# stripe/rainier

Hardware: NVIDIA H100
Metric: leapfrog_steps_x_chains_per_sec (higher is better)
Workload: dtype f64

## Files before the change

rainier_b200/csrc/rn_sampler.cuh:

```cuda
#ifndef RN_SAMPLER_CUH
#define RN_SAMPLER_CUH


#if RN_MASS_MAX >= 1
#define RN_TS_NMASS RN_N
#else
#define RN_TS_NMASS 0
#endif
#if RN_ENABLE_EHMC
#define RN_TS_NSNAP RN_N
#else
#define RN_TS_NSNAP 0
#endif
#ifndef RN_TS_RESTORE
#define RN_TS_RESTORE 0
#endif
#if RN_TS_RESTORE
#define RN_TS_NREST (2 * RN_N + 1)
#else
#define RN_TS_NREST 0
#endif
#define RN_TS_P 0
#define RN_TS_MASS (RN_N + 1)
#define RN_TS_SNAP (RN_TS_MASS + RN_TS_NMASS)
#define RN_TS_STAT (RN_TS_SNAP + RN_TS_NSNAP)
#define RN_TS_HOT (RN_TS_STAT + 5)
#define RN_TS_REST (RN_TS_HOT + 4)
#define RN_TS_DOUBLES (RN_TS_REST + RN_TS_NREST)
#define RN_TS_INTS 10
struct RnTs {
  double* d;
  int* i;
  unsigned bs;
};
#ifdef RN_HOST_EMULATION
static thread_local double rn_ts_mem_d[RN_TS_DOUBLES];
static thread_local int rn_ts_mem_i[RN_TS_INTS];
RN_DEVICE RnTs rn_ts_get() { return RnTs{rn_ts_mem_d, rn_ts_mem_i, 1u}; }
#define RN_STCS(ptr, v) (*(ptr) = (v))
#else
extern __shared__ double rn_ts_mem[];
RN_DEVICE RnTs rn_ts_get() {
  RnTs T;
#ifdef RN_BLOCK_DIM
  T.bs = RN_BLOCK_DIM;
#else
  T.bs = blockDim.x;
#endif
  T.d = rn_ts_mem + threadIdx.x;
  T.i = (int*)(rn_ts_mem + (size_t)RN_TS_DOUBLES * blockDim.x) + threadIdx.x;
  return T;
}
#define RN_STCS(ptr, v) __stcs((ptr), (v))
#endif
#define RN_TSD(slot) T.d[(unsigned)(slot) * T.bs]
#define RN_TSI(slot) T.i[(unsigned)(slot) * T.bs]
#ifndef RN_X_P_REGS
#define RN_X_P_REGS 1
#endif
#ifndef RN_X_NORMALS
#define RN_X_NORMALS 3
#endif
#define RN_Z(i) RN_TSD(RN_TS_P + (i))
#if RN_X_P_REGS
#define RN_P(i) s.p[i]
#else
#define RN_P(i) RN_TSD(RN_TS_P + (i))
#endif
#define RN_MASSD(i) RN_TSD(RN_TS_MASS + (i))
#define RN_SNAP_P(i) RN_TSD(RN_TS_SNAP + (i))
#define RN_ST_E_MEAN RN_TSD(RN_TS_STAT + 0)
#define RN_ST_E_RAW RN_TSD(RN_TS_STAT + 1)
#define RN_ST_TRANS2 RN_TSD(RN_TS_STAT + 2)
#define RN_ST_GRADS RN_TSD(RN_TS_STAT + 3)
#define RN_ST_STEPS RN_TSD(RN_TS_STAT + 4)
#define RN_ST_ITERS RN_TSI(0)
#define RN_ST_ACCEPTED RN_TSI(1)
#define RN_ST_E_N RN_TSI(2)
#define RN_ST_RING_I(r) RN_TSI(3 + (r))
#define RN_ST_RING_FULL(r) RN_TSI(6 + (r))
#define RN_TS_PREV_H RN_TSD(RN_TS_HOT + 2)
#define RN_TS_START_H RN_TSD(RN_TS_HOT + 3)
#define RN_REST_Q(i) RN_TSD(RN_TS_REST + (i))
#define RN_REST_G(i) RN_TSD(RN_TS_REST + RN_N + (i))
#define RN_REST_U RN_TSD(RN_TS_REST + 2 * RN_N)

struct RnIt {
  int grads, steps, err;
};

RN_DEVICE RnRng rn_rng_unpark(const RnTs& T) {
  RnRng r;
  r.seed = rn_d2ll(RN_TSD(RN_TS_HOT + 0));
  r.nng = RN_TSD(RN_TS_HOT + 1);
  r.have = RN_TSI(9);
  return r;
}
RN_DEVICE void rn_rng_park(const RnTs& T, const RnRng& r) {
  RN_TSD(RN_TS_HOT + 0) = rn_ll2d(r.seed);
  RN_TSD(RN_TS_HOT + 1) = r.nng;
  RN_TSI(9) = r.have;
}

RN_DEVICE void rn_ring_add(const RnArgs& A, int c, const RnTs& T, int which, double value) {
  int i = RN_ST_RING_I(which) + 1;
  if (i == A.stats_window) {
    RN_ST_RING_FULL(which) = 1;
    i = 0;
  }
  RN_ST_RING_I(which) = i;
  RN_STCS(&RN_AT(A.st_rings, which * A.stats_window + i, c), value);
}

struct RnPQ {
  double q[RN_N], g[RN_N];
  double U;
#if RN_X_P_REGS
  double p[RN_N];
#endif
};

RN_DEVICE double rn_velocity_i(const RnArgs& A, int c, const RnTs& T, const RnPQ& s, int kind, int i) {
  (void)s;
  (void)T;
  (void)A;
  (void)c;
#if RN_MASS_MAX >= 2
  if (kind == 2) {
    double y = 0.0;
    for (int j = 0; j < RN_N; j++) y += RN_P(j) * RN_AT(A.mass, i * RN_N + j, c);
    return y;
  }
#endif
#if RN_MASS_MAX >= 1
  if (kind == 1) return RN_P(i) * RN_MASSD(i);
#endif
  (void)kind;
  return RN_P(i);
}

RN_DEVICE double rn_energy(const RnArgs& A, int c, const RnTs& T, const RnPQ& s, int kind, double U) {
  double k = 0.0;
#if RN_MASS_MAX >= 2
  if (kind == 2) {
    for (int i = 0; i < RN_N; i++) k += (rn_velocity_i(A, c, T, s, 2, i) * RN_P(i));
    return U + k / 2.0;
  }
#endif
  RN_UNROLL
  for (int i = 0; i < RN_N; i++) k += (rn_velocity_i(A, c, T, s, kind, i) * RN_P(i));
  return U + k / 2.0;
}

RN_DEVICE double rn_log_accept(double deltaH) {
  if (deltaH != deltaH) return -RN_INF;
  return rn_jmin0(-deltaH);
}


RN_DEVICE void rn_update(const RnArgs& A, RnPQ& s, RnIt& S) {
  double dens;
  rn_density(s.q, dens, s.g, A.data, S.err);
  s.U = dens * -1;
  S.grads += 1;
}
RN_DEVICE void rn_full_ps(const RnTs& T, RnPQ& s, double stepSize, RnIt& S) {
  (void)T;
  S.grads += 1;
  RN_UNROLL
  for (int i = 0; i < RN_N; i++) RN_P(i) += stepSize * s.g[i];
}
RN_DEVICE void rn_new_qs(const RnArgs& A, int c, const RnTs& T, int kind, RnPQ& s, double stepSize) {
#if RN_MASS_MAX >= 2
  if (kind == 2) {
    for (int i = 0; i < RN_N; i++) s.q[i] += (stepSize * rn_velocity_i(A, c, T, s, 2, i));
    return;
  }
#endif
  RN_UNROLL
  for (int i = 0; i < RN_N; i++) s.q[i] += (stepSize * rn_velocity_i(A, c, T, s, kind, i));
}
RN_DEVICE void rn_leapfrog(const RnArgs& A, int c, const RnTs& T, int kind, RnPQ& s, int l, double stepSize, RnIt& S) {
  rn_full_ps(T, s, stepSize / 2.0, S);
  for (int i = 0;;) {
    rn_new_qs(A, c, T, kind, s, stepSize);
    rn_update(A, s, S);
    if (++i >= l) break;
    rn_full_ps(T, s, stepSize, S);
  }
  rn_full_ps(T, s, stepSize / 2.0, S);
}
RN_DEVICE void rn_take_steps(const RnArgs& A, int c, const RnTs& T, int kind, RnPQ& s, int l, double stepSize, RnIt& S) {
  rn_ring_add(A, c, T, 0, stepSize);
  rn_leapfrog(A, c, T, kind, s, l, stepSize, S);
  S.steps += l;
}

RN_DEVICE void rn_draw_normals(const RnTs& T, RnRng& rng) {
#if RN_X_NORMALS == 2
  for (int i = 0; i < RN_N; i++) RN_Z(i) = rn_normal(rng);
  return;
#endif
  int i0 = 0;
  if (rng.have) {
    rng.have = 0;
    RN_Z(0) = rng.nng;
    i0 = 1;
  }
  const int npairs = (RN_N - i0 + 1) / 2;
#ifndef RN_X_POLAR2
#define RN_X_POLAR2 1
#endif
#if RN_X_POLAR2
  for (int k = 0; k < npairs;) {
    double a1, a2, b1, b2;
    rn_i64 seed4, seed8;
    rn_polar_attempt2(rng, a1, a2, b1, b2, seed4, seed8);
    const double sa = a1 * a1 + a2 * a2, sb = b1 * b1 + b2 * b2;
    const bool oka = !(sa >= 1 || sa == 0);
    const int kb = k + (oka ? 1 : 0);
    const bool needb = kb < npairs;
    const bool okb = needb && !(sb >= 1 || sb == 0);
    if (oka) {
      RN_Z(i0 + 2 * k) = a1;
      RN_Z(i0 + 2 * k + 1) = a2;
    }
    if (okb) {
      RN_Z(i0 + 2 * kb) = b1;
      RN_Z(i0 + 2 * kb + 1) = b2;
    }
    rng.seed = needb ? seed8 : seed4;
    k = kb + (okb ? 1 : 0);
  }
#else
  for (int k = 0; k < npairs;) {
    double v1, v2;
    rn_polar_attempt(rng, v1, v2);
    const double s = v1 * v1 + v2 * v2;
    if (!(s >= 1 || s == 0)) {
      RN_Z(i0 + 2 * k) = v1;
      RN_Z(i0 + 2 * k + 1) = v2;
      k += 1;
    }
  }
#endif
#if RN_X_NORMALS == 4 && RN_X_SPEC && !defined(RN_FAST_MATH) && !(defined(RN_X_LIBM_PLAIN) && RN_X_LIBM_PLAIN)
#pragma unroll 1
  for (int k = 0; k < npairs; k += 2) {
    const int ia = i0 + 2 * k, ib = i0 + 2 * (k + 1 < npairs ? k + 1 : k);
    const double a1 = RN_Z(ia), a2 = RN_Z(ia + 1), b1 = RN_Z(ib), b2 = RN_Z(ib + 1);
    const double sa = a1 * a1 + a2 * a2, sb = b1 * b1 + b2 * b2;
    bool oka, okb;
    double la = rn_strict_log_try(sa, oka), lb = rn_strict_log_try(sb, okb);
    if (!(oka && okb)) {
      la = rn_strict_log_full(sa);
      lb = rn_strict_log_full(sb);
    }
    const double ma = rn_sqrt_nc(rn_div_nc(-2 * la, sa)), mb = rn_sqrt_nc(rn_div_nc(-2 * lb, sb));
    RN_Z(ia) = a1 * ma;
    if (ia + 1 < RN_N) {
      RN_Z(ia + 1) = a2 * ma;
    } else {
      rng.nng = a2 * ma;
      rng.have = 1;
    }
    RN_Z(ib) = b1 * mb;
    if (ib + 1 < RN_N) {
      RN_Z(ib + 1) = b2 * mb;
    } else {
      rng.nng = b2 * mb;
      rng.have = 1;
    }
  }
  return;
#endif
#if RN_X_NORMALS == 1
#pragma unroll 1
#elif RN_X_NORMALS == 3
#pragma unroll 2
#endif
  for (int k = 0; k < npairs; k++) {
    const int i = i0 + 2 * k;
    const double v1 = RN_Z(i), v2 = RN_Z(i + 1);
    const double s = v1 * v1 + v2 * v2;
    const double multiplier = rn_polar_multiplier(s);
    RN_Z(i) = v1 * multiplier;
    if (i + 1 < RN_N) {
      RN_Z(i + 1) = v2 * multiplier;
    } else {
      rng.nng = v2 * multiplier;
      rng.have = 1;
    }
  }
}

RN_DEVICE void rn_initialize_ps(const RnArgs& A, int c, const RnTs& T, RnPQ& s, int kind, RnRng& rng) {
  (void)A;
  (void)c;
  (void)kind;
  (void)s;
  rn_draw_normals(T, rng);
#if RN_X_P_REGS
  RN_UNROLL
  for (int i = 0; i < RN_N; i++) s.p[i] = RN_Z(i);
#endif
#if RN_MASS_MAX >= 2
  if (kind == 2) {
    int i = RN_N - 1;
    int m = ((i + 1) * (i + 2)) / 2 - 1;
    while (i >= 0) {
      int j = RN_N - 1;
      double dot = 0.0;
      while (j > i) {
        dot += RN_Z(j) * RN_AT(A.chol, m, c);
        j -= 1;
        m -= 1;
      }
      RN_Z(i) = (RN_Z(i) - dot) / RN_AT(A.chol, m, c);
      i -= 1;
      m -= 1;
    }
#if RN_X_P_REGS
    for (int k = 0; k < RN_N; k++) s.p[k] = RN_Z(k);
#endif
    return;
  }
#endif
#if RN_MASS_MAX >= 1
  if (kind == 1) {
    RN_UNROLL
    for (int i = 0; i < RN_N; i++) RN_P(i) = RN_P(i) / sqrt(RN_MASSD(i));
    return;
  }
#endif
}

RN_DEVICE void rn_load_mass(const RnArgs& A, int c, const RnTs& T, int kind) {
  (void)A;
  (void)c;
  (void)T;
  (void)kind;
#if RN_MASS_MAX >= 1
  if (kind == 1) {
    RN_UNROLL
    for (int i = 0; i < RN_N; i++) RN_MASSD(i) = RN_AT(A.mass, i, c);
  }
#endif
}

RN_DEVICE void rn_load_stats(const RnArgs& A, int c, const RnTs& T) {
  RN_ST_GRADS = rn_ll2d(A.st_grads[c]);
  RN_ST_STEPS = rn_ll2d(A.st_steps[c]);
  RN_ST_ITERS = A.st_iters[c];
  RN_ST_ACCEPTED = A.st_accepted[c];
  RN_ST_E_MEAN = RN_AT(A.st_energy, 0, c);
  RN_ST_E_RAW = RN_AT(A.st_energy, 1, c);
  RN_ST_TRANS2 = RN_AT(A.st_energy, 2, c);
  RN_ST_E_N = A.st_energy_n[c];
  for (int r = 0; r < 3; r++) {
    RN_ST_RING_I(r) = RN_AT(A.st_ring_i, r, c);
    RN_ST_RING_FULL(r) = RN_AT(A.st_ring_full, r, c);
  }
}
RN_DEVICE void rn_store_stats(const RnArgs& A, int c, const RnTs& T, int err) {
  A.st_grads[c] = rn_d2ll(RN_ST_GRADS);
  A.st_steps[c] = rn_d2ll(RN_ST_STEPS);
  A.st_iters[c] = RN_ST_ITERS;
  A.st_accepted[c] = RN_ST_ACCEPTED;
  if (err) A.st_err[c] |= err;
  RN_AT(A.st_energy, 0, c) = RN_ST_E_MEAN;
  RN_AT(A.st_energy, 1, c) = RN_ST_E_RAW;
  RN_AT(A.st_energy, 2, c) = RN_ST_TRANS2;
  A.st_energy_n[c] = RN_ST_E_N;
  for (int r = 0; r < 3; r++) {
    RN_AT(A.st_ring_i, r, c) = RN_ST_RING_I(r);
    RN_AT(A.st_ring_full, r, c) = RN_ST_RING_FULL(r);
  }
}
RN_DEVICE void rn_fold(const RnTs& T, RnIt& S) {
  RN_ST_GRADS = rn_ll2d(rn_d2ll(RN_ST_GRADS) + (rn_i64)S.grads);
  RN_ST_STEPS = rn_ll2d(rn_d2ll(RN_ST_STEPS) + (rn_i64)S.steps);
  S.grads = 0;
  S.steps = 0;
}

RN_GLOBAL void rn_k_init(const RnArgs A) {
  const int c = (int)(blockIdx.x * blockDim.x + threadIdx.x);
  if (c >= A.chains) return;
  const RnTs T = rn_ts_get();
  RnRng rng;
  rng.seed = A.rng_seed[c];
  rng.nng = A.rng_nng[c];
  rng.have = A.rng_have[c];
  rn_load_stats(A, c, T);
  RnIt S;
  S.grads = 0;
  S.steps = 0;
  S.err = 0;

  RnPQ s;
  rn_draw_normals(T, rng);
  RN_UNROLL
  for (int i = 0; i < RN_N; i++) s.q[i] = RN_Z(i);
  rn_update(A, s, S);
  double cq[RN_N], cg[RN_N];
  const double cU = s.U;
  RN_UNROLL
  for (int i = 0; i < RN_N; i++) {
    cq[i] = s.q[i];
    cg[i] = s.g[i];
  }
  rn_initialize_ps(A, c, T, s, 0, rng);
  RN_UNROLL
  for (int i = 0; i < RN_N; i++) RN_AT(A.params, i, c) = RN_P(i);

  double stepSize;
  if (A.step_tuner == 0) {
    const double H0 = rn_energy(A, c, T, s, 0, cU);
    stepSize = 1.0;
    double lap;
    rn_leapfrog(A, c, T, 0, s, 1, stepSize, S);
    lap = rn_log_accept(rn_energy(A, c, T, s, 0, s.U) - H0);
    const double exponent = (lap > -RN_LN2) ? 1.0 : -1.0;
    const double doubleOrHalf = (exponent > 0) ? 2.0 : 0.5;
#if RN_STEP_POOL
    int log2Step = 0;
#endif
    while (stepSize != 0.0 && (exponent * lap > -exponent * RN_LN2)) {
      stepSize *= doubleOrHalf;
#if RN_STEP_POOL
      log2Step += (exponent > 0) ? 1 : -1;
#endif
      RN_UNROLL
      for (int i = 0; i < RN_N; i++) {
        RN_P(i) = RN_AT(A.params, i, c);
        s.q[i] = cq[i];
        s.g[i] = cg[i];
      }
      s.U = cU;
      rn_leapfrog(A, c, T, 0, s, 1, stepSize, S);
      lap = rn_log_accept(rn_energy(A, c, T, s, 0, s.U) - H0);
    }
    rn_da_apply(stepSize, RN_AT(A.da, 1, c), RN_AT(A.da, 2, c), RN_AT(A.da, 3, c), RN_AT(A.da, 4, c), A.da_iter[c]);
#if RN_STEP_POOL
    rn_pool_add_initial_step(A.step_acc, log2Step);
#endif
  } else {
    stepSize = A.static_step;
  }
  RN_AT(A.da, 0, c) = stepSize;

  RN_UNROLL
  for (int i = 0; i < RN_N; i++) {
    RN_AT(A.params, RN_N + i, c) = cq[i];
    RN_AT(A.grad, i, c) = cg[i];
  }
  RN_AT(A.params, 2 * RN_N, c) = cU;
  A.rng_seed[c] = rng.seed;
  A.rng_nng[c] = rng.nng;
  A.rng_have[c] = rng.have;
  rn_fold(T, S);
  rn_store_stats(A, c, T, S.err);
}

enum { RN_P_IN_PARAMS = 0, RN_P_IN_REGS = 1, RN_P_IN_Z = 2 };
RN_DEVICE void rn_store_momentum(const RnArgs& A, int c, const RnTs& T, const RnPQ& s, int where) {
  (void)s;
  if (where == RN_P_IN_PARAMS) return;
  RN_UNROLL
  for (int i = 0; i < RN_N; i++) RN_AT(A.params, i, c) = where == RN_P_IN_REGS ? RN_P(i) : RN_Z(i);
}

template <int PHASE>
RN_DEVICE void rn_iterate(const RnArgs& A) {
  const int c = A.chain_begin + (int)(blockIdx.x * blockDim.x + threadIdx.x);
  if (c >= A.chain_end) return;
  const RnTs T = rn_ts_get();
  {
    RnRng rng;
    rng.seed = A.rng_seed[c];
    rng.nng = A.rng_nng[c];
    rng.have = A.rng_have[c];
    rn_rng_park(T, rng);
  }
  rn_load_stats(A, c, T);
  RnIt S;
  S.grads = 0;
  S.steps = 0;
  S.err = 0;
#if RN_MASS_MAX >= 1
  int kind = A.mass_kind;
#else
  constexpr int kind = 0;
#endif
  rn_load_mass(A, c, T, kind);

  double stepSize = RN_AT(A.da, 0, c);
  if (PHASE == 1 && A.step_tuner == 0) stepSize = rn_exp(RN_AT(A.da, 2, c));
  int win_size = A.win_size, win_i = A.win_i, win_j = A.win_j, est_samples = A.est_samples;
#if RN_ENABLE_EHMC
  int ring_i = 0, ring_full = 0;
  if (A.sampler == 1) {
    ring_i = A.ring_i[c];
    ring_full = A.ring_full[c];
  }
#endif
  bool havePrevH = false;

#ifndef RN_X_KEEP_STATE
#define RN_X_KEEP_STATE 1
#endif
#define RN_KEEP_P_LATE (RN_X_KEEP_STATE && RN_X_P_REGS)
#define RN_REST_ON_CHIP (RN_X_KEEP_STATE && RN_TS_RESTORE)
#if RN_REST_ON_CHIP
#define RN_X0(i) RN_REST_Q(i)
  int p_at = RN_P_IN_PARAMS;
#else
#define RN_X0(i) RN_AT(A.params, RN_N + (i), c)
#endif
  RnPQ s;
#if RN_X_KEEP_STATE
  RN_UNROLL
  for (int i = 0; i < RN_N; i++) {
    s.q[i] = RN_AT(A.params, RN_N + i, c);
    s.g[i] = RN_AT(A.grad, i, c);
  }
  s.U = RN_AT(A.params, 2 * RN_N, c);
#endif

  for (int it = 0; it < A.n_iter; it++) {
#if RN_X_KEEP_STATE
    const double cU = s.U;
#else
    const double cU = RN_AT(A.params, 2 * RN_N, c);
#endif
    if (!havePrevH) {
      RN_UNROLL
      for (int i = 0; i < RN_N; i++) RN_P(i) = RN_AT(A.params, i, c);
      RN_TS_PREV_H = rn_energy(A, c, T, s, kind, cU);
    }
    {
      RnRng rng = rn_rng_unpark(T);
      rn_initialize_ps(A, c, T, s, kind, rng);
      rn_rng_park(T, rng);
    }
#if RN_X_KEEP_STATE
    if (!(RN_KEEP_P_LATE && kind == 0)) {
      RN_UNROLL
      for (int i = 0; i < RN_N; i++) RN_AT(A.params, i, c) = RN_P(i);
    }
#else
    RN_UNROLL
    for (int i = 0; i < RN_N; i++) {
      RN_AT(A.params, i, c) = RN_P(i);
      s.q[i] = RN_AT(A.params, RN_N + i, c);
      s.g[i] = RN_AT(A.grad, i, c);
    }
#endif
    s.U = cU;
    RN_TS_START_H = rn_energy(A, c, T, s, kind, cU);
#if RN_REST_ON_CHIP
    RN_UNROLL
    for (int i = 0; i < RN_N; i++) {
      RN_REST_Q(i) = s.q[i];
      RN_REST_G(i) = s.g[i];
    }
    RN_REST_U = cU;
#endif
    const double usedStep = stepSize;

    if (A.sampler == 0) {
      rn_take_steps(A, c, T, kind, s, A.n_steps, stepSize, S);
    }
#if RN_ENABLE_EHMC
    else {
      bool count = false;
      if (PHASE == 0 && !ring_full) count = true;
      else if (PHASE == 0) {
        RnRng rng = rn_rng_unpark(T);
        count = rn_uniform(rng) < A.p_count;
        rn_rng_park(T, rng);
      }
      if (count) {
        RnPQ snap;
        int l = 0;
        for (;;) {
          double out = 0.0;
          RN_UNROLL
          for (int i = 0; i < RN_N; i++) out += (s.q[i] - RN_X0(i)) * RN_P(i);
          const bool uturn = (out != out) ? true : (out < 0);
          if (uturn || !(l < A.max_steps)) break;
          l += 1;
          rn_take_steps(A, c, T, kind, s, 1, stepSize, S);
          if (l == A.min_steps) {
            snap = s;
#if !(RN_X_P_REGS)
            RN_UNROLL
            for (int i = 0; i < RN_N; i++) RN_SNAP_P(i) = RN_P(i);
#endif
          }
        }
        if (l < A.min_steps) {
          rn_take_steps(A, c, T, kind, s, A.min_steps - l, stepSize, S);
        } else {
          s = snap;
#if !(RN_X_P_REGS)
          RN_UNROLL
          for (int i = 0; i < RN_N; i++) RN_P(i) = RN_SNAP_P(i);
#endif
        }
        ring_i += 1;
        if (ring_i == A.buf_size) ring_full = 1;
        ring_i = ring_i % A.buf_size;
        RN_AT(A.ring, ring_i, c) = (double)l;
      } else {
        RnRng rng = rn_rng_unpark(T);
        const int idx = ring_full ? rn_rng_int(rng, A.buf_size) : rn_rng_int(rng, ring_i + 1);
        rn_rng_park(T, rng);
        const int nsteps = rn_d2i(RN_AT(A.ring, idx, c));
        rn_take_steps(A, c, T, kind, s, nsteps, stepSize, S);
      }
    }
#endif

    const double endH = rn_energy(A, c, T, s, kind, s.U);
    const double startH = RN_TS_START_H;
    const double deltaH = endH - startH;
    const double a = rn_log_accept(deltaH);
    bool accept;
    {
      RnRng rng = rn_rng_unpark(T);
      accept = a > rn_log(rn_uniform(rng));
      rn_rng_park(T, rng);
    }
    double eH;
    if (accept) {
#if RN_REST_ON_CHIP
      p_at = RN_P_IN_REGS;
#else
      RN_UNROLL
      for (int i = 0; i < RN_N; i++) {
        RN_AT(A.params, i, c) = RN_P(i);
        RN_AT(A.params, RN_N + i, c) = s.q[i];
        RN_AT(A.grad, i, c) = s.g[i];
      }
      RN_AT(A.params, 2 * RN_N, c) = s.U;
#endif
      eH = endH;
      RN_ST_ACCEPTED += 1;
    } else {
#if RN_REST_ON_CHIP
      RN_UNROLL
      for (int i = 0; i < RN_N; i++) {
        s.q[i] = RN_REST_Q(i);
        s.g[i] = RN_REST_G(i);
      }
      s.U = RN_REST_U;
      p_at = (RN_KEEP_P_LATE && kind == 0) ? RN_P_IN_Z : RN_P_IN_PARAMS;
#else
      RN_UNROLL
      for (int i = 0; i < RN_N; i++) s.q[i] = RN_AT(A.params, RN_N + i, c);
#if RN_X_KEEP_STATE
      RN_UNROLL
      for (int i = 0; i < RN_N; i++) s.g[i] = RN_AT(A.grad, i, c);
      s.U = RN_AT(A.params, 2 * RN_N, c);
      if (RN_KEEP_P_LATE && kind == 0) {
        RN_UNROLL
        for (int i = 0; i < RN_N; i++) RN_AT(A.params, i, c) = RN_Z(i);
      }
#endif
#endif
      eH = startH;
    }
    {
      const int e_n = RN_ST_E_N + 1;
      RN_ST_E_N = e_n;
      double e_mean = RN_ST_E_MEAN;
      const double oldDiff = eH - e_mean;
      e_mean += (oldDiff / (double)e_n);
      RN_ST_E_MEAN = e_mean;
      const double newDiff = eH - e_mean;
      RN_ST_E_RAW += oldDiff * newDiff;
      const double d = eH - RN_TS_PREV_H;
      RN_ST_TRANS2 += d * d;
    }
    RN_TS_PREV_H = eH;
    havePrevH = true;
    RN_ST_ITERS += 1;
    rn_ring_add(A, c, T, 1, rn_exp(a));
    rn_ring_add(A, c, T, 2, (double)S.grads);

    if (A.trace) {
      double* tr = A.trace + (size_t)it * 4 * (size_t)A.chains;
      tr[0 * (size_t)A.chains + c] = a;
      tr[1 * (size_t)A.chains + c] = accept ? 1.0 : 0.0;
      tr[2 * (size_t)A.chains + c] = usedStep;
      tr[3 * (size_t)A.chains + c] = (double)S.steps;
    }
    rn_fold(T, S);

    if (PHASE == 0) {
#if RN_STEP_POOL
      if (A.step_tuner == 0) rn_pool_add(A.step_acc + it, rn_pool_quantise(rn_exp(a)));
#else
      if (A.step_tuner == 0) {
        const double newAcceptanceProb = rn_exp(a);
        const int daIter = A.da_iter[c] + 1;
        A.da_iter[c] = daIter;
        const double avgErrorMultiplier = 1.0 / ((double)daIter + 10);
        const double stepSizeMultiplier = rn_pow((double)daIter, -0.75);
        const double avgError = ((1.0 - avgErrorMultiplier) * RN_AT(A.da, 3, c) + (avgErrorMultiplier * (A.delta - newAcceptanceProb)));
        RN_AT(A.da, 3, c) = avgError;
        const double logStepSize = (RN_AT(A.da, 4, c) - (avgError * sqrt((double)daIter) / 0.05));
        RN_AT(A.da, 1, c) = logStepSize;
        RN_AT(A.da, 2, c) = (stepSizeMultiplier * logStepSize + (1.0 - stepSizeMultiplier) * RN_AT(A.da, 2, c));
        stepSize = rn_exp(logStepSize);
      }
#endif
#if RN_MASS_MAX >= 1
      if (A.mass_tuner == 1 || A.mass_tuner == 2) {
        win_j += 1;
        if (A.adaptation == 1) {
          if (RN_IN_WINDOW(A, win_j)) {
            win_i += 1;
#if RN_MASS_POOL
            double oldDiff[RN_N], newDiff[RN_N];
            RN_UNROLL
            for (int i = 0; i < RN_N; i++) newDiff[i] = rn_variance_update(A, c, i, s.q[i], win_i, oldDiff[i]);
            for (int j = 0; j < RN_N; j++)
              for (int k = 0; k < RN_N; k++) RN_AT(A.est_cov, j * RN_N + k, c) += newDiff[j] * oldDiff[k];
#else
            RN_UNROLL
            for (int i = 0; i < RN_N; i++) {
              double oldDiff;
              rn_variance_update(A, c, i, s.q[i], win_i, oldDiff);
            }
#endif
            if (win_i == win_size) {
              win_i = 0;
              win_size = rn_d2i(win_size * A.win_expansion);
            }
          }
        } else if (RN_IN_WINDOW(A, win_j)) {
          win_i += 1;
          est_samples += 1;
#if RN_MASS_MAX >= 2
          double oldDiff[RN_N], newDiff[RN_N];
          RN_UNROLL
          for (int i = 0; i < RN_N; i++) newDiff[i] = rn_variance_update(A, c, i, s.q[i], est_samples, oldDiff[i]);
#else
          RN_UNROLL
          for (int i = 0; i < RN_N; i++) {
            double oldDiff;
            rn_variance_update(A, c, i, s.q[i], est_samples, oldDiff);
          }
#endif
#if RN_MASS_MAX >= 2
          if (A.mass_tuner == 2) {
            for (int j = 0; j < RN_N; j++)
              for (int k = 0; k < RN_N; k++) RN_AT(A.est_cov, j * RN_N + k, c) += newDiff[j] * oldDiff[k];
          }
#endif
          if (win_i == win_size) {
            win_i = 0;
            win_size = rn_d2i(win_size * A.win_expansion);
            havePrevH = false;
#if RN_REST_ON_CHIP
            rn_store_momentum(A, c, T, s, p_at);
            p_at = RN_P_IN_PARAMS;
#endif
            if (A.mass_tuner == 1) {
              kind = 1;
              RN_UNROLL
              for (int i = 0; i < RN_N; i++) {
                const double v = RN_AT(A.est_raw, i, c) / (double)est_samples;
                if (v == 0.0) S.err |= 2;
                RN_MASSD(i) = v;
                RN_AT(A.mass, i, c) = v;
                RN_AT(A.est_mean, i, c) = 0.0;
                RN_AT(A.est_raw, i, c) = 0.0;
              }
            }
#if RN_MASS_MAX >= 2
            else {
              kind = 2;
              const double z = (double)(est_samples - 1);
              for (int i = 0; i < RN_N * RN_N; i++) {
                const double v = RN_AT(A.est_cov, i, c) / z;
                if (v == 0.0) S.err |= 2;
                RN_AT(A.mass, i, c) = v;
                RN_AT(A.est_cov, i, c) = 0.0;
              }
              for (int i = 0; i < RN_N; i++) {
                RN_AT(A.est_mean, i, c) = 0.0;
                RN_AT(A.est_raw, i, c) = 0.0;
              }
              double lower[(RN_N * (RN_N + 1)) / 2];
              rn_cholesky_upper(A, c, lower, 1);
            }
#endif
#if !RN_STEP_POOL
            if (A.step_tuner == 0)
              stepSize = rn_da_reset(RN_AT(A.da, 1, c), RN_AT(A.da, 2, c), RN_AT(A.da, 3, c), RN_AT(A.da, 4, c), A.da_iter[c]);
#endif
          }
        }
      }
#endif
    } else if (A.samples) {
      double* out = A.samples + (size_t)it * RN_N * (size_t)A.chains;
      RN_UNROLL
      for (int i = 0; i < RN_N; i++) RN_STCS(&out[(size_t)i * (size_t)A.chains + c], s.q[i]);
    }
  }

#if RN_REST_ON_CHIP
  rn_store_momentum(A, c, T, s, p_at);
  RN_UNROLL
  for (int i = 0; i < RN_N; i++) {
    RN_AT(A.params, RN_N + i, c) = s.q[i];
    RN_AT(A.grad, i, c) = s.g[i];
  }
  RN_AT(A.params, 2 * RN_N, c) = s.U;
#endif
  if (PHASE == 0) RN_AT(A.da, 0, c) = stepSize;
#if RN_ENABLE_EHMC
  if (A.sampler == 1) {
    A.ring_i[c] = ring_i;
    A.ring_full[c] = ring_full;
  }
#endif
  {
    const RnRng rng = rn_rng_unpark(T);
    A.rng_seed[c] = rng.seed;
    A.rng_nng[c] = rng.nng;
    A.rng_have[c] = rng.have;
  }
  rn_store_stats(A, c, T, S.err);
}
RN_GLOBAL void rn_k_warmup(const RnArgs A) { rn_iterate<0>(A); }
RN_GLOBAL void rn_k_iter(const RnArgs A) { rn_iterate<1>(A); }
#define RN_K_WARMUP rn_k_warmup

RN_GLOBAL void rn_k_density(const double* RN_RESTRICT qin, double* RN_RESTRICT out, const double* data, int* err,
                            int chains) {
  const int c = (int)(blockIdx.x * blockDim.x + threadIdx.x);
  if (c >= chains) return;
  double q[RN_N], g[RN_N], dens;
  RN_UNROLL
  for (int i = 0; i < RN_N; i++) q[i] = qin[(size_t)i * chains + c];
  int e = 0;
  rn_density(q, dens, g, data, e);
  out[c] = dens;
  RN_UNROLL
  for (int i = 0; i < RN_N; i++) out[(size_t)(i + 1) * chains + c] = g[i];
#ifdef RN_HOST_EMULATION
  if (e) *err |= e;
#else
  if (e) atomicOr(err, e);
#endif
}

#endif
```

Before: 29.01 billion.

## Draw acceptance uniform with momentum normals and batch its log into polar loop

Switches the default normal-generation path to the paired strict-log variant. For plain HMC it also draws the Metropolis uniform right after the momentum normals and computes its log in the spare slot of the paired-log loop. This is meant to remove a separate uniform draw and log call at accept time. The catch is that the RNG draw order changes, so the random streams and sampled chains differ from the previous code for the same seed.

```diff
diff --git a/rainier_b200/csrc/rn_sampler.cuh b/rainier_b200/csrc/rn_sampler.cuh
--- a/rainier_b200/csrc/rn_sampler.cuh
+++ b/rainier_b200/csrc/rn_sampler.cuh
@@ -59,7 +59,7 @@
 #define RN_X_P_REGS 1
 #endif
 #ifndef RN_X_NORMALS
-#define RN_X_NORMALS 3
+#define RN_X_NORMALS 4
 #endif
 #define RN_Z(i) RN_TSD(RN_TS_P + (i))
 #if RN_X_P_REGS
@@ -196,9 +196,10 @@
   S.steps += l;
 }
 
-RN_DEVICE void rn_draw_normals(const RnTs& T, RnRng& rng) {
+RN_DEVICE void rn_draw_normals(const RnTs& T, RnRng& rng, bool with_u, double& logu) {
 #if RN_X_NORMALS == 2
   for (int i = 0; i < RN_N; i++) RN_Z(i) = rn_normal(rng);
+  if (with_u) logu = rn_log(rn_uniform(rng));
   return;
 #endif
   int i0 = 0;
@@ -244,19 +245,22 @@
     }
   }
 #endif
+  const double u = with_u ? rn_uniform(rng) : 0.0;
 #if RN_X_NORMALS == 4 && RN_X_SPEC && !defined(RN_FAST_MATH) && !(defined(RN_X_LIBM_PLAIN) && RN_X_LIBM_PLAIN)
 #pragma unroll 1
   for (int k = 0; k < npairs; k += 2) {
-    const int ia = i0 + 2 * k, ib = i0 + 2 * (k + 1 < npairs ? k + 1 : k);
+    const bool last_odd = k + 1 >= npairs;
+    const bool slot_u = with_u && last_odd;
+    const int ia = i0 + 2 * k, ib = i0 + 2 * (last_odd ? k : k + 1);
     const double a1 = RN_Z(ia), a2 = RN_Z(ia + 1), b1 = RN_Z(ib), b2 = RN_Z(ib + 1);
-    const double sa = a1 * a1 + a2 * a2, sb = b1 * b1 + b2 * b2;
+    const double sa = a1 * a1 + a2 * a2, sb = slot_u ? u : b1 * b1 + b2 * b2;
     bool oka, okb;
     double la = rn_strict_log_try(sa, oka), lb = rn_strict_log_try(sb, okb);
     if (!(oka && okb)) {
       la = rn_strict_log_full(sa);
       lb = rn_strict_log_full(sb);
     }
-    const double ma = rn_sqrt_nc(rn_div_nc(-2 * la, sa)), mb = rn_sqrt_nc(rn_div_nc(-2 * lb, sb));
+    const double ma = rn_sqrt_nc(rn_div_nc(-2 * la, sa));
     RN_Z(ia) = a1 * ma;
     if (ia + 1 < RN_N) {
       RN_Z(ia + 1) = a2 * ma;
@@ -264,6 +268,11 @@
       rng.nng = a2 * ma;
       rng.have = 1;
     }
+    if (slot_u) {
+      logu = lb;
+      continue;
+    }
+    const double mb = rn_sqrt_nc(rn_div_nc(-2 * lb, sb));
     RN_Z(ib) = b1 * mb;
     if (ib + 1 < RN_N) {
       RN_Z(ib + 1) = b2 * mb;
@@ -272,6 +281,7 @@
       rng.have = 1;
     }
   }
+  if (with_u && npairs % 2 == 0) logu = rn_log(u);
   return;
 #endif
 #if RN_X_NORMALS == 1
@@ -292,14 +302,15 @@
       rng.have = 1;
     }
   }
-}
-
-RN_DEVICE void rn_initialize_ps(const RnArgs& A, int c, const RnTs& T, RnPQ& s, int kind, RnRng& rng) {
+  if (with_u) logu = rn_log(u);
+}
+
+RN_DEVICE void rn_initialize_ps(const RnArgs& A, int c, const RnTs& T, RnPQ& s, int kind, RnRng& rng, bool with_u, double& logu) {
   (void)A;
   (void)c;
   (void)kind;
   (void)s;
-  rn_draw_normals(T, rng);
+  rn_draw_normals(T, rng, with_u, logu);
 #if RN_X_P_REGS
   RN_UNROLL
   for (int i = 0; i < RN_N; i++) s.p[i] = RN_Z(i);
@@ -399,7 +410,8 @@
   S.err = 0;
 
   RnPQ s;
-  rn_draw_normals(T, rng);
+  double unused;
+  rn_draw_normals(T, rng, false, unused);
   RN_UNROLL
   for (int i = 0; i < RN_N; i++) s.q[i] = RN_Z(i);
   rn_update(A, s, S);
@@ -410,7 +422,7 @@
     cq[i] = s.q[i];
     cg[i] = s.g[i];
   }
-  rn_initialize_ps(A, c, T, s, 0, rng);
+  rn_initialize_ps(A, c, T, s, 0, rng, false, unused);
   RN_UNROLL
   for (int i = 0; i < RN_N; i++) RN_AT(A.params, i, c) = RN_P(i);
 
@@ -539,9 +551,10 @@
       for (int i = 0; i < RN_N; i++) RN_P(i) = RN_AT(A.params, i, c);
       RN_TS_PREV_H = rn_energy(A, c, T, s, kind, cU);
     }
+    double logu = 0.0;
     {
       RnRng rng = rn_rng_unpark(T);
-      rn_initialize_ps(A, c, T, s, kind, rng);
+      rn_initialize_ps(A, c, T, s, kind, rng, !RN_ENABLE_EHMC || A.sampler == 0, logu);
       rn_rng_park(T, rng);
     }
 #if RN_X_KEEP_STATE
@@ -627,12 +640,14 @@
     const double startH = RN_TS_START_H;
     const double deltaH = endH - startH;
     const double a = rn_log_accept(deltaH);
-    bool accept;
-    {
+    bool accept = a > logu;
+#if RN_ENABLE_EHMC
+    if (A.sampler == 1) {
       RnRng rng = rn_rng_unpark(T);
       accept = a > rn_log(rn_uniform(rng));
       rn_rng_park(T, rng);
     }
+#endif
     double eH;
     if (accept) {
 #if RN_REST_ON_CHIP
```

Result: faster. 29.31 billion, median of 6 (+1.1%).
